# danieleschmidt/Graph-Hypernetwork-Forge

Measured on AMD Instinct MI355X. Metric: edges/s (HyperGNN forward), higher is better.
Workload: dtype f32; 1 GPU; synthetic uniform KG 1M nodes / 10M edges / 64 rel, hidden 128, L=3 (BASELINE config 3); nodes=1000000, edges=10000000, relations=64, hidden_dim=128, layers=3, text_dim=64, plan=cached (warm), launch=one C-ABI call per kernel, parallelism=single GPU

## Files before the change

graph-hypernetwork-forge_amd/csrc/message_bx.hip:

```cpp
#include "common.h"

#include <type_traits>

namespace ghf {

typedef float f32x4 __attribute__((ext_vector_type(4)));
typedef int i32x4 __attribute__((ext_vector_type(4)));
typedef int i32x2 __attribute__((ext_vector_type(2)));
typedef float f32x2 __attribute__((ext_vector_type(2)));
typedef _Float16 f16x8 __attribute__((ext_vector_type(8)));
typedef _Float16 f16x4 __attribute__((ext_vector_type(4)));
typedef __attribute__((address_space(3))) void* lptr_t;

template <class T>
__device__ __forceinline__ const T* bx_at(const void* base, uint32_t byte_off) {
    return (const T*)((const char*)base + byte_off);
}

__device__ __forceinline__ int lds_ld_b32(unsigned addr) {
    int v;
    asm volatile("ds_read_b32 %0, %1\n\ts_waitcnt lgkmcnt(0)" : "=&v"(v) : "v"(addr) : "memory");
    return v;
}
__device__ __forceinline__ void lds_ld_b32_x2(unsigned a0, unsigned a1, int& v0, int& v1) {
    asm volatile("ds_read_b32 %0, %2\n\tds_read_b32 %1, %3\n\ts_waitcnt lgkmcnt(0)" : "=&v"(v0), "=&v"(v1) : "v"(a0), "v"(a1) : "memory");
}
__device__ __forceinline__ void lds_ld_b32_x6(const unsigned (&a)[6], int (&v)[6]) {
    asm volatile("ds_read_b32 %0, %6\n\tds_read_b32 %1, %7\n\tds_read_b32 %2, %8\n\tds_read_b32 %3, %9\n\tds_read_b32 %4, %10\n\t"
                 "ds_read_b32 %5, %11\n\ts_waitcnt lgkmcnt(0)"
                 : "=&v"(v[0]), "=&v"(v[1]), "=&v"(v[2]), "=&v"(v[3]), "=&v"(v[4]), "=&v"(v[5])
                 : "v"(a[0]), "v"(a[1]), "v"(a[2]), "v"(a[3]), "v"(a[4]), "v"(a[5]) : "memory");
}
__device__ __forceinline__ void lds_ld_b32_x10(const unsigned (&a)[10], int (&v)[10]) {
    asm volatile("ds_read_b32 %0, %10\n\tds_read_b32 %1, %11\n\tds_read_b32 %2, %12\n\tds_read_b32 %3, %13\n\tds_read_b32 %4, %14\n\t"
                 "ds_read_b32 %5, %15\n\tds_read_b32 %6, %16\n\tds_read_b32 %7, %17\n\tds_read_b32 %8, %18\n\tds_read_b32 %9, %19\n\t"
                 "s_waitcnt lgkmcnt(0)"
                 : "=&v"(v[0]), "=&v"(v[1]), "=&v"(v[2]), "=&v"(v[3]), "=&v"(v[4]), "=&v"(v[5]), "=&v"(v[6]), "=&v"(v[7]), "=&v"(v[8]), "=&v"(v[9])
                 : "v"(a[0]), "v"(a[1]), "v"(a[2]), "v"(a[3]), "v"(a[4]), "v"(a[5]), "v"(a[6]), "v"(a[7]), "v"(a[8]), "v"(a[9]) : "memory");
}
__device__ __forceinline__ void lds_ld_b64_x2(unsigned a0, unsigned a1, f32x2& v0, f32x2& v1) {
    asm volatile("ds_read_b64 %0, %2\n\tds_read_b64 %1, %3\n\ts_waitcnt lgkmcnt(0)" : "=&v"(v0), "=&v"(v1) : "v"(a0), "v"(a1) : "memory");
}
__device__ __forceinline__ void lds_st_b32(unsigned addr, int v) { asm volatile("ds_write_b32 %0, %1" ::"v"(addr), "v"(v) : "memory"); }
__device__ __forceinline__ void lds_st_b64(unsigned addr, f32x2 v) { asm volatile("ds_write_b64 %0, %1" ::"v"(addr), "v"(v) : "memory"); }
__device__ __forceinline__ void lds_st_b128(unsigned addr, f32x4 v) { asm volatile("ds_write_b128 %0, %1" ::"v"(addr), "v"(v) : "memory"); }
#define BX_LGKM0() asm volatile("s_waitcnt lgkmcnt(0)" ::: "memory")
__device__ __forceinline__ int opaque_lane(int lane) {
    int z;
    asm volatile("v_mov_b32 %0, 0" : "=v"(z));
    return lane + z;
}

__device__ __forceinline__ int fresh_lane() {
    int z;
    asm volatile("v_mov_b32 %0, 0" : "=v"(z));
    return (int)__builtin_amdgcn_mbcnt_hi(~0u, __builtin_amdgcn_mbcnt_lo(~0u, (unsigned)z));
}

template <class T> __device__ __forceinline__ T bx_tail_ld(const T* p) { return __builtin_nontemporal_load(p); }
template <class T> __device__ __forceinline__ void bx_tail_st(T* p, T v) { __builtin_nontemporal_store(v, p); }
#define BX_IDX_WAIT "s_nop 3\n\t"
constexpr int BX_AD = 2, BX_TGB = 3;

template <int D> struct BxCfg;
template <> struct BxCfg<128> {
    static constexpr int NPW = 96, CR = 76;
    static constexpr int BN = 4 * NPW;
    static constexpr int MTC = (CR + 15) / 16;
    static constexpr bool DEFER = true;
    static constexpr size_t LDS = (size_t)4 * 2 * CR * 256 + 4 * (4 * 16 * MTC + 4) * 4 + 1024 + 512 + 64;
};
template <> struct BxCfg<64> {
    static constexpr int NPW = 48, CR = 64;
    static constexpr int BN = 4 * NPW;
    static constexpr int MTC = (CR + 15) / 16;
    static constexpr bool DEFER = false;
    static constexpr size_t LDS = (size_t)4 * 2 * CR * 128 + 4 * (4 * 16 * MTC + 4) * 4 + 1024 + 512 + 64;
};

typedef float f32x32 __attribute__((ext_vector_type(32)));
typedef float f32x16 __attribute__((ext_vector_type(16)));
#define BX_PIN_128(s) "+{v[64:95]}"(s[0]), "+{v[96:127]}"(s[1]), "+{v[128:159]}"(s[2]), "+{v[160:191]}"(s[3]), "+{v[192:223]}"(s[4]), "+{v[224:255]}"(s[5])
#define BX_PIN_64(s) "+{v[64:79]}"(s[0]), "+{v[80:95]}"(s[1]), "+{v[96:111]}"(s[2])

struct BxChunk { int r; int e0; int rows; };

template <int GB_, int NV_> struct BxTailSt {
    static constexpr int GB = GB_, NV = NV_;
    f32x4 x[GB_][NV_];
    int deg[GB_];
    float gm[4 * NV_], bt[4 * NV_];
};
constexpr int BX_TCG = 8;

template <int D, int SKIP>
__global__ __launch_bounds__(512, D == 64 ? 4 : 2) void message_bx_kernel(
    const float* __restrict__ h, const void* __restrict__ h_split, int64_t N, const uint32_t* __restrict__ sorted_key,
    const int32_t* __restrict__ sorted_src, const int32_t* __restrict__ chunk_tab,
    const int32_t* __restrict__ item_tab, int64_t item0, float* __restrict__ partial,
    const int32_t* __restrict__ indeg, int R,
    const void* __restrict__ Wsplit, const float* __restrict__ bias,
    const float* __restrict__ gamma, const float* __restrict__ beta, float eps,
    int64_t row0, int64_t row_end, float* __restrict__ h_out, void* __restrict__ h_split_out, int no_tail,
    int32_t* __restrict__ range_flag, float* __restrict__ agg_out) {
    using C = BxCfg<D>;
    constexpr bool SWAP1 = SKIP == 1;
    constexpr int skip = SWAP1 ? 2 : SKIP;
    constexpr int P0_IDS = SWAP1 ? 3 : 2;
    constexpr int P0_HALF = SWAP1 ? 1 : 0;
    constexpr int BN = C::BN, MTC = C::MTC, CR = C::CR, NPW = C::NPW;
    constexpr bool DEFER = C::DEFER;
    constexpr int NWV = 8, TW = 4;
    constexpr int KS = D / 32;
    constexpr int NKS = 2 * KS;
    constexpr int NT = D / 16;
    constexpr int NTW = NT / TW;
    constexpr int NPL = 2;
    constexpr int ROWB = D * 2;
    constexpr int PLANE = CR * ROWB;
    constexpr int TILE = NPL * PLANE;
    constexpr int HROW = NPL * D * 2;
    constexpr int CRP = 16 * MTC;
    constexpr int MSTR = 4 * CRP + 4;
    constexpr int PL = D / 64;
    constexpr int TUP = D == 128 ? 32 : 16;
    constexpr int NSV = NPW * PL / TUP;
    constexpr int RPP = 1024 / ROWB;
    constexpr int LPR = 64 / RPP;
    constexpr int RBN = CR / RPP;
    constexpr int CPL = D / 16;
    constexpr int RBW = (RBN + TW - 1) / TW;
    constexpr int RPH = (CR + TW - 1) / TW;
    static_assert((NTW == 2 || NTW == 1) && CR % RPP == 0 && RPH <= 64 && NPW * TW == BN && (NPW * PL) % TUP == 0 && NPW * PL <= 192 &&
                      NPW % 2 == 0 && (BN / 2) % 4 == 0 && CR <= 128 && NSV <= 6 && (D == 128 || D == 64), "bad config");
    auto akey = [](int row) -> int { return D == 128 ? (row & 15) : ((row >> 1) & 7); };
    constexpr unsigned META_OFF = 4 * TILE,
                       DUMMY_OFF = META_OFF + 4 * MSTR * 4, ZERO_OFF = DUMMY_OFF + 1024,
                       FLAG_OFF = ZERO_OFF + 512;
    auto tile_of = [](int j) -> unsigned { return (unsigned)(j & 3) * (unsigned)TILE; };

    extern __shared__ __attribute__((aligned(16))) char smem[];
    const unsigned lds0 = (unsigned)(size_t)(lptr_t)smem;

    const int tid = threadIdx.x, lane = tid & 63;
    const int w = __builtin_amdgcn_readfirstlane(tid >> 6);
    const bool helper = w >= TW;
    const int tw = w & 3;
    const int q = lane >> 4, c16 = lane & 15;
    const i32x4 item = *(const i32x4*)(item_tab + 4 * (size_t)(item0 + blockIdx.x));
    const int64_t blk = __builtin_amdgcn_readfirstlane(item[0]);
    const int slot = __builtin_amdgcn_readfirstlane(item[3]);
    const int64_t node0 = blk * BN;
    const int nrows = (int)((row_end - node0) < BN ? (row_end - node0) : BN);
    const uint32_t seg0 = (uint32_t)(blk * R);
    const int c_begin = __builtin_amdgcn_readfirstlane(item[1]);
    const int c_end = __builtin_amdgcn_readfirstlane(item[2]);
    const int nchunks = c_end - c_begin;
    int vzero;
    asm volatile("v_mov_b32 %0, 0" : "=v"(vzero));

    auto load_desc = [&](int k) -> i32x2 {
        const int c = c_begin + (k < nchunks ? k : 0) + vzero;
        return *bx_at<i32x2>(chunk_tab, (uint32_t)c * 8u);
    };
    auto decode = [&](i32x2 d) -> BxChunk {
        const int w0 = __builtin_amdgcn_readfirstlane(d[0]), w1 = __builtin_amdgcn_readfirstlane(d[1]);
        return BxChunk{w1 >> 8, w0, w1 & 127};
    };
    auto meta_off = [&](int j) -> unsigned { return META_OFF + (unsigned)(j & 3) * (MSTR * 4); };
    const uint32_t hsc_off = (uint32_t)((uint64_t)N * HROW);

    constexpr int HN = BN / 2, HPW = NPW / 2;
    auto tail_half = [&](int half, auto gb_c) __attribute__((always_inline)) {
        const float* acc_lds = (const float*)smem;
        constexpr int CS = 64;
        const int sub = lane >> 4, c0 = 4 * (lane & 15);
        constexpr int NV = CPL / 4;
        auto node_of = [&](int v) -> int { return (v / HPW) * NPW + half * HPW + (v % HPW); };
        auto row_sum = [&](float v) -> float {
            v += dpp_take<0xB1, 0xF>(v);
            v += dpp_take<0x4E, 0xF>(v);
            v += dpp_take<0x141, 0xF>(v);
            v += dpp_take<0x140, 0xF>(v);
            return v;
        };
        auto row_max = [&](float v) -> float {
            v = fmaxf(v, dpp_take<0xB1, 0xF>(v));
            v = fmaxf(v, dpp_take<0x4E, 0xF>(v));
            v = fmaxf(v, dpp_take<0x141, 0xF>(v));
            v = fmaxf(v, dpp_take<0x140, 0xF>(v));
            return v;
        };
        constexpr int NG = HN / 4;
        if (slot >= 0) {
            float* __restrict__ ps = partial + (size_t)slot * BN * D;
            for (int g = w; g < NG; g += NWV) {
                const int v = 4 * g + sub;
                float* __restrict__ o = ps + (size_t)node_of(v) * D + c0;
#pragma unroll
                for (int i = 0; i < NV; ++i) *(f32x4*)(o + CS * i) = *(const f32x4*)(acc_lds + v * D + c0 + CS * i);
            }
            return;
        }
        float gm[CPL], bt[CPL];
#pragma unroll
        for (int c = 0; c < CPL; ++c) {
            gm[c] = no_tail ? 1.f : gamma[c0 + CS * (c >> 2) + (c & 3)];
            bt[c] = no_tail ? 0.f : beta[c0 + CS * (c >> 2) + (c & 3)];
        }
        constexpr int GB = decltype(gb_c)::value;
        for (int g0 = w; g0 < NG; g0 += NWV * GB) {
            f32x4 x[GB][NV];
            float inv[GB];
            int deg[GB];
#pragma unroll
            for (int gb = 0; gb < GB; ++gb) {
                const int g = g0 + gb * NWV;
                const int nl = node_of(4 * (g < NG ? g : NG - 1) + sub);
                const int64_t node = node0 + (nl < nrows ? nl : nrows - 1);
                deg[gb] = indeg[node];
                const float* __restrict__ hp = h + (size_t)node * D + c0;
#pragma unroll
                for (int i = 0; i < NV; ++i)
                    x[gb][i] = (no_tail && !(no_tail & GHF_FLAG_ADD_H)) ? (f32x4){0.f, 0.f, 0.f, 0.f} : bx_tail_ld((const f32x4*)(hp + CS * i));
            }
            __builtin_amdgcn_sched_barrier(0);
#pragma unroll
            for (int gb = 0; gb < GB; ++gb) inv[gb] = (no_tail & GHF_FLAG_RAW_SUM) ? 1.0f : 1.0f / (float)(deg[gb] > 1 ? deg[gb] : 1);
#pragma unroll
            for (int gb = 0; gb < GB; ++gb) {
                const int g = g0 + gb * NWV;
                const int v = 4 * (g < NG ? g : NG - 1) + sub;
                const int nl = node_of(v);
                const bool live = g < NG && nl < nrows;
                f32x4 a[NV];
#pragma unroll
                for (int i = 0; i < NV; ++i) a[i] = *(const f32x4*)(acc_lds + v * D + c0 + CS * i);
                if (agg_out && live) {
                    float* __restrict__ o = agg_out + (size_t)(node0 + nl) * D + c0;
#pragma unroll
                    for (int i = 0; i < NV; ++i) bx_tail_st((f32x4*)(o + CS * i), a[i] * inv[gb]);
                }
                float y[CPL];
                float s = 0.f;
#pragma unroll
                for (int c = 0; c < CPL; ++c) {
                    const float av = a[c >> 2][c & 3] * inv[gb];
                    y[c] = no_tail ? av + x[gb][c >> 2][c & 3] : fmaxf(av + x[gb][c >> 2][c & 3], 0.f);
                    s += y[c];
                }
                if (!no_tail) {
                    const float mean = row_sum(s) * (1.0f / D);
                    float var = 0.f;
#pragma unroll
                    for (int c = 0; c < CPL; ++c) { const float t = y[c] - mean; var += t * t; }
                    const float rstd = 1.0f / sqrtf(row_sum(var) * (1.0f / D) + eps);
#pragma unroll
                    for (int c = 0; c < CPL; ++c) y[c] = (y[c] - mean) * rstd * gm[c] + bt[c];
                }
                float up = 1.f;
                if (h_split_out) {
                    float mx = 0.f;
#pragma unroll
                    for (int c = 0; c < CPL; ++c) mx = fmaxf(mx, fabsf(y[c]));
                    const int sh = split2h_shift(row_max(mx));
                    up = pow2f(sh);
                    if ((lane & 15) == 0 && live) *(float*)((char*)h_split_out + (size_t)hsc_off + (size_t)(node0 + nl) * 4) = pow2f(-sh);
                }
                if (live) {
                    float* __restrict__ o = h_out + (size_t)(node0 + nl) * D + c0;
#pragma unroll
                    for (int i = 0; i < NV; ++i) bx_tail_st((f32x4*)(o + CS * i), (f32x4){y[4 * i], y[4 * i + 1], y[4 * i + 2], y[4 * i + 3]});
                    if (h_split_out) {
                        _Float16* __restrict__ sp = (_Float16*)h_split_out + (size_t)(node0 + nl) * (NPL * D) + c0;
                        _Float16 hi[CPL], lo[CPL];
#pragma unroll
                        for (int c = 0; c < CPL; ++c) split2h(y[c] * up, hi[c], lo[c]);
                        if constexpr (CPL == 8 && CS == 4) {
                            *(f16x8*)sp = (f16x8){hi[0], hi[1], hi[2], hi[3], hi[4], hi[5], hi[6], hi[7]};
                            *(f16x8*)(sp + D) = (f16x8){lo[0], lo[1], lo[2], lo[3], lo[4], lo[5], lo[6], lo[7]};
                        } else if constexpr (CPL == 8) {
#pragma unroll
                            for (int i = 0; i < 2; ++i) {
                                bx_tail_st((f16x4*)(sp + CS * i), (f16x4){hi[4 * i], hi[4 * i + 1], hi[4 * i + 2], hi[4 * i + 3]});
                                bx_tail_st((f16x4*)(sp + D + CS * i), (f16x4){lo[4 * i], lo[4 * i + 1], lo[4 * i + 2], lo[4 * i + 3]});
                            }
                        } else {
                            bx_tail_st((f16x4*)sp, (f16x4){hi[0], hi[1], hi[2], hi[3]});
                            bx_tail_st((f16x4*)(sp + D), (f16x4){lo[0], lo[1], lo[2], lo[3]});
                        }
                    }
                }
                if (h_split_out) {
                    int tiny = 0, nz = 0;
#pragma unroll
                    for (int c = 0; c < CPL; ++c) { tiny += range_tiny(y[c] * up); nz += y[c] != 0.f; }
                    if (__ballot(tiny != 0)) {
                        tiny = (int)row_sum((float)tiny);
                        nz = (int)row_sum((float)nz);
                        if ((lane & 15) == 0 && live) range_raise(range_flag, GHF_RANGE_ROWS, tiny, nz);
                    }
                }
            }
        }
    };

    auto tail_issue = [&](int half, auto& st, int gfirst, auto gend_c) __attribute__((always_inline)) {
        using St = typename std::remove_reference<decltype(st)>::type;
        constexpr int GB = St::GB, NV = St::NV, CS = 64;
        static_assert(NV * 4 == CPL && 4 * GB <= decltype(gend_c)::value, "one batch holds all of the wave's groups");
        if (slot >= 0) return;
        const int tl = fresh_lane(), sub = tl >> 4, c0 = 4 * (tl & 15);
        const bool no_x = no_tail && !(no_tail & GHF_FLAG_ADD_H);
        const __amdgpu_buffer_rsrc_t rsG = __builtin_amdgcn_make_buffer_rsrc((void*)gamma, 0, no_tail ? 0 : D * 4, 0x00020000);
        const __amdgpu_buffer_rsrc_t rsB = __builtin_amdgcn_make_buffer_rsrc((void*)beta, 0, no_tail ? 0 : D * 4, 0x00020000);
        const __amdgpu_buffer_rsrc_t rsX = __builtin_amdgcn_make_buffer_rsrc(
            (void*)h, 0, no_x ? 0 : (int)(uint32_t)((uint64_t)N * D * 4), 0x00020000);
#pragma unroll
        for (int c = 0; c < CPL; ++c) {
            st.gm[c] = __builtin_bit_cast(float, __builtin_amdgcn_raw_buffer_load_b32(rsG, (c0 + CS * (c >> 2) + (c & 3)) * 4, 0, 0));
            st.bt[c] = __builtin_bit_cast(float, __builtin_amdgcn_raw_buffer_load_b32(rsB, (c0 + CS * (c >> 2) + (c & 3)) * 4, 0, 0));
        }
#pragma unroll
        for (int gb = 0; gb < GB; ++gb) {
            const int v = 4 * (gfirst + 4 * gb) + sub;
            const int nl = (v / HPW) * NPW + half * HPW + (v % HPW);
            const int64_t node = node0 + (nl < nrows ? nl : nrows - 1);
            st.deg[gb] = indeg[node];
#pragma unroll
            for (int i = 0; i < NV; ++i)
                st.x[gb][i] = __builtin_bit_cast(f32x4, __builtin_amdgcn_raw_buffer_load_b128(
                    rsX, (int)(((uint32_t)node * D + c0 + CS * i) * 4u), 0, 2 ));
        }
        __builtin_amdgcn_sched_barrier(0);
    };
    auto tail_rows = [&](int half, auto& st, int gfirst, auto gend_c) __attribute__((always_inline)) {
        using St = typename std::remove_reference<decltype(st)>::type;
        constexpr int GB = St::GB, NV = St::NV, gend = decltype(gend_c)::value, CS = 64;
        __builtin_amdgcn_s_waitcnt(0x0F70);
        const float* acc_lds = (const float*)smem;
        const int tl = fresh_lane(), sub = tl >> 4, c0 = 4 * (tl & 15);
        auto node_of = [&](int v) -> int { return (v / HPW) * NPW + half * HPW + (v % HPW); };
        auto row_sum = [&](float v) -> float {
            v += dpp_take<0xB1, 0xF>(v);
            v += dpp_take<0x4E, 0xF>(v);
            v += dpp_take<0x141, 0xF>(v);
            v += dpp_take<0x140, 0xF>(v);
            return v;
        };
        auto row_max = [&](float v) -> float {
            v = fmaxf(v, dpp_take<0xB1, 0xF>(v));
            v = fmaxf(v, dpp_take<0x4E, 0xF>(v));
            v = fmaxf(v, dpp_take<0x141, 0xF>(v));
            v = fmaxf(v, dpp_take<0x140, 0xF>(v));
            return v;
        };
        if (slot >= 0) {
            float* __restrict__ ps = partial + (size_t)slot * BN * D;
            for (int g = gfirst; g < gend; g += 4) {
                const int v = 4 * g + sub;
                float* __restrict__ o = ps + (size_t)node_of(v) * D + c0;
#pragma unroll
                for (int i = 0; i < NV; ++i) *(f32x4*)(o + CS * i) = *(const f32x4*)(acc_lds + v * D + c0 + CS * i);
            }
            return;
        }
        float inv[GB];
#pragma unroll
        for (int gb = 0; gb < GB; ++gb) inv[gb] = (no_tail & GHF_FLAG_RAW_SUM) ? 1.0f : 1.0f / (float)(st.deg[gb] > 1 ? st.deg[gb] : 1);
#pragma unroll
        for (int gb = 0; gb < GB; ++gb) {
            const int v = 4 * (gfirst + 4 * gb) + sub;
            const int nl = node_of(v);
            const bool live = nl < nrows;
            f32x4 a[NV];
#pragma unroll
            for (int i = 0; i < NV; ++i) a[i] = *(const f32x4*)(acc_lds + v * D + c0 + CS * i);
            if (agg_out && live) {
                float* __restrict__ o = agg_out + (size_t)(node0 + nl) * D + c0;
#pragma unroll
                for (int i = 0; i < NV; ++i) bx_tail_st((f32x4*)(o + CS * i), a[i] * inv[gb]);
            }
            float y[CPL];
            float s = 0.f;
#pragma unroll
            for (int c = 0; c < CPL; ++c) {
                const float av = a[c >> 2][c & 3] * inv[gb];
                y[c] = no_tail ? av + st.x[gb][c >> 2][c & 3] : fmaxf(av + st.x[gb][c >> 2][c & 3], 0.f);
                s += y[c];
            }
            if (!no_tail) {
                const float mean = row_sum(s) * (1.0f / D);
                float var = 0.f;
#pragma unroll
                for (int c = 0; c < CPL; ++c) { const float t = y[c] - mean; var += t * t; }
                const float rstd = 1.0f / sqrtf(row_sum(var) * (1.0f / D) + eps);
#pragma unroll
                for (int c = 0; c < CPL; ++c) y[c] = (y[c] - mean) * rstd * st.gm[c] + st.bt[c];
            }
            float up = 1.f;
            if (h_split_out) {
                float mx = 0.f;
#pragma unroll
                for (int c = 0; c < CPL; ++c) mx = fmaxf(mx, fabsf(y[c]));
                const int sh = split2h_shift(row_max(mx));
                up = pow2f(sh);
                if ((tl & 15) == 0 && live) *(float*)((char*)h_split_out + (size_t)hsc_off + (size_t)(node0 + nl) * 4) = pow2f(-sh);
            }
            if (live) {
                float* __restrict__ o = h_out + (size_t)(node0 + nl) * D + c0;
#pragma unroll
                for (int i = 0; i < NV; ++i) bx_tail_st((f32x4*)(o + CS * i), (f32x4){y[4 * i], y[4 * i + 1], y[4 * i + 2], y[4 * i + 3]});
                if (h_split_out) {
                    _Float16* __restrict__ sp = (_Float16*)h_split_out + (size_t)(node0 + nl) * (NPL * D) + c0;
                    _Float16 hi[CPL], lo[CPL];
#pragma unroll
                    for (int c = 0; c < CPL; ++c) split2h(y[c] * up, hi[c], lo[c]);
#pragma unroll
                    for (int i = 0; i < NV; ++i) {
                        bx_tail_st((f16x4*)(sp + CS * i), (f16x4){hi[4 * i], hi[4 * i + 1], hi[4 * i + 2], hi[4 * i + 3]});
                        bx_tail_st((f16x4*)(sp + D + CS * i), (f16x4){lo[4 * i], lo[4 * i + 1], lo[4 * i + 2], lo[4 * i + 3]});
                    }
                }
            }
            if (h_split_out) {
                int tiny = 0, nz = 0;
#pragma unroll
                for (int c = 0; c < CPL; ++c) { tiny += range_tiny(y[c] * up); nz += y[c] != 0.f; }
                if (__ballot(tiny != 0)) {
                    tiny = (int)row_sum((float)tiny);
                    nz = (int)row_sum((float)nz);
                    if ((tl & 15) == 0 && live) range_raise(range_flag, GHF_RANGE_ROWS, tiny, nz);
                }
            }
        }
    };
    auto tail_barrier = [&]() __attribute__((always_inline)) {
        BX_LGKM0();
        __builtin_amdgcn_s_barrier();
        asm volatile("" ::: "memory");
    };
    constexpr int TNG = BN / 2 / 4;
    constexpr int TCG = BX_TCG, THG = TNG / 4 - TCG;
    static_assert(D != 128 || (TNG % 4 == 0 && TCG >= 1 && THG >= 1 && 9 * THG + 2 * CPL <= 96),
                  "the helpers' operands of a half fit the registers its dump freed");
    std::integral_constant<int, TNG> c_tng;
    std::integral_constant<int, 4 * TCG> c_cend;

    if (helper) {
        typename std::conditional<D == 128, f32x32, f32x16>::type sm[NSV];
#pragma unroll
        for (int k = 0; k < NSV; ++k)
#pragma unroll
            for (int i = 0; i < TUP; ++i) sm[k][i] = 0.f;
        if constexpr (D == 128) asm volatile("" : BX_PIN_128(sm)); else asm volatile("" : BX_PIN_64(sm));
        const int hw = tw;
        const __amdgpu_buffer_rsrc_t rsH = __builtin_amdgcn_make_buffer_rsrc((void*)h_split, 0, (int)hsc_off, 0x00020000);
        struct Words { int src; int key; };
        struct Scales { float u; float v; };
        auto load_words = [&](const BxChunk& c, int ln) -> Words {
            const int mrow = hw * RPH + (ln < RPH ? ln : RPH - 1);
            const int rc = mrow < c.rows ? mrow : c.rows - 1;
            const uint32_t eo = (uint32_t)(c.e0 + rc) * 4u;
            return Words{*bx_at<int>(sorted_src, eo), *bx_at<int>(sorted_key, eo)};
        };
        auto dst_of = [&](const BxChunk& c, const Words& wd) -> uint32_t {
            const uint32_t kbase = (seg0 + (uint32_t)c.r) * (uint32_t)BN;
            return (uint32_t)node0 + ((uint32_t)wd.key - kbase);
        };
        auto load_scales = [&](const BxChunk& c, const Words& wd) -> Scales {
            const uint32_t nu = (uint32_t)(wd.src & SRC_MASK), nv = dst_of(c, wd);
            return Scales{*bx_at<float>(h_split, hsc_off + nu * 4u), *bx_at<float>(h_split, hsc_off + nv * 4u)};
        };
        auto publish = [&](int j, const BxChunk& c, const Words& wd, const Scales& sc, int ln) {
            const unsigned m = lds0 + meta_off(j);
            const int mrow = hw * RPH + (ln < RPH ? ln : RPH - 1);
            if (ln < RPH && mrow < CRP) {
                lds_st_b32(m + 4 * mrow, __float_as_int(sc.u));
                lds_st_b32(m + 4 * (CRP + mrow), __float_as_int(sc.v));
                lds_st_b32(m + 4 * (2 * CRP + mrow), wd.src & SRC_MASK);
                lds_st_b32(m + 4 * (3 * CRP + mrow), (int)dst_of(c, wd));
            }
            if (hw == 0 && ln == 0) lds_st_b32(m + 4 * (4 * CRP), c.rows);
        };
        static_assert(RBW <= 6, "ids of a tile: one batched read");
        auto id_addr = [&](int j, int which , int i, int lane) -> unsigned {
            return lds0 + meta_off(j) + 4 * (which * CRP) + 4 * (RPP * (hw + TW * (i < RBW ? i : 0)) + lane / LPR);
        };
        auto dma_ids = [&](int j, int which, int lane, int (&id)[6]) {
            unsigned ia[6];
#pragma unroll
            for (int i = 0; i < 6; ++i) ia[i] = id_addr(j, which, i, lane);
            lds_ld_b32_x6(ia, id);
        };
        auto dma_issue = [&](unsigned tile_off, int rows, int lane, const int (&id)[6]) {
#pragma unroll
            for (int i_ = 0; i_ < RBW; ++i_) {
                const int i = i_;
                const int rb = hw + TW * i, row = RPP * rb + lane / LPR;
                if (RPP * rb >= rows) continue;
                const int g = (lane & (LPR - 1)) ^ akey(row);
                const int voff = row < rows ? (int)((uint32_t)id[i] * (uint32_t)HROW) + (g << 4) : (int)0xFFFFF000u;
                const unsigned dst = rb < RBN ? tile_off + (unsigned)rb * 1024u : DUMMY_OFF;
#pragma unroll
                for (int pl = 0; pl < NPL; ++pl) {
                    const unsigned d = __builtin_amdgcn_readfirstlane(dst + (rb < RBN ? pl * PLANE : 0));
                    __builtin_amdgcn_raw_ptr_buffer_load_lds(rsH, (lptr_t)(smem + d), 16, voff + pl * ROWB, 0, 0, 0);
                }
            }
        };
        auto dma_tile = [&](unsigned tile_off, int j, int which, const BxChunk& c, int lane) {
            int id[6];
            dma_ids(j, which, lane, id);
            dma_issue(tile_off, c.rows, lane, id);
        };
        struct FoldPlan { int n0, n1, ra, cnt; };
        auto fold_plan = [&](int j, int rows, int lane) __attribute__((always_inline)) -> FoldPlan {
            const unsigned dd = lds0 + meta_off(j) + 4 * (3 * CRP);
            int d0, d1;
            lds_ld_b32_x2(dd + 4 * lane, dd + 4 * (lane + 64 < CRP ? lane + 64 : CRP - 1), d0, d1);
            const int base = (int)node0 + hw * NPW;
            const int n0 = d0 - base, n1 = d1 - base;
            const unsigned long long q0 = __ballot(lane < rows && (unsigned)n0 < (unsigned)NPW);
            const unsigned long long q1 = __ballot(lane + 64 < rows && (unsigned)n1 < (unsigned)NPW);
            const int cnt = __builtin_popcountll(q0) + __builtin_popcountll(q1);
            const int ra = q0 ? (int)__builtin_ctzll(q0) : 64 + (q1 ? (int)__builtin_ctzll(q1) : 0);
            return FoldPlan{n0, n1, ra, cnt};
        };
        auto fold_rows = [&](int j, const FoldPlan& fp, int lane) __attribute__((always_inline)) {
            const unsigned Y = lds0 + tile_of(j - 1);
            const int ra = fp.ra, cnt = fp.cnt;
            const unsigned zrow = lds0 + ZERO_OFF + (unsigned)(PL * 4 * lane), lb = (unsigned)(PL * 4 * lane);
            typedef typename std::conditional<D == 128, f32x2, float>::type yv_t;
            constexpr int FB = 4;
            auto issue = [&](yv_t (&y)[FB], int r0) __attribute__((always_inline)) {
                unsigned a[FB];
#pragma unroll
                for (int i = 0; i < FB; ++i) {
                    const int rr = ra + r0 + i;
                    a[i] = r0 + i < cnt ? Y + (unsigned)rr * (D * 4) + (lb ^ (unsigned)(((rr >> 2) & 1) << 7)) : zrow;
                }
                if constexpr (D == 128)
                    asm volatile("ds_read_b64 %0, %4\n\tds_read_b64 %1, %5\n\tds_read_b64 %2, %6\n\tds_read_b64 %3, %7"
                                 : "=&v"(y[0]), "=&v"(y[1]), "=&v"(y[2]), "=&v"(y[3]) : "v"(a[0]), "v"(a[1]), "v"(a[2]), "v"(a[3]) : "memory");
                else
                    asm volatile("ds_read_b32 %0, %4\n\tds_read_b32 %1, %5\n\tds_read_b32 %2, %6\n\tds_read_b32 %3, %7"
                                 : "=&v"(y[0]), "=&v"(y[1]), "=&v"(y[2]), "=&v"(y[3]) : "v"(a[0]), "v"(a[1]), "v"(a[2]), "v"(a[3]) : "memory");
            };
            auto add_rows = [&](yv_t (&y)[FB], int r0, bool behind) __attribute__((always_inline)) {
                if (behind) asm volatile("s_waitcnt lgkmcnt(4)" : "+v"(y[0]), "+v"(y[1]), "+v"(y[2]), "+v"(y[3])::"memory");
                else asm volatile("s_waitcnt lgkmcnt(0)" : "+v"(y[0]), "+v"(y[1]), "+v"(y[2]), "+v"(y[3])::"memory");
                int ix[FB];
#pragma unroll
                for (int i = 0; i < FB; ++i) {
                    const int rr = ra + r0 + i;
                    const int a = __builtin_amdgcn_readlane(fp.n0, rr & 63), b = __builtin_amdgcn_readlane(fp.n1, rr & 63);
                    ix[i] = r0 + i < cnt ? PL * (rr < 64 ? a : b) : 0;
                }
                int keep;
#define BX_ROW128(i) "s_set_gpr_idx_idx %[i" #i "]\n\tv_pk_add_f32 v[64:65], %[y" #i "], v[64:65]\n\t"
#define BX_ROW64(i) "s_set_gpr_idx_idx %[i" #i "]\n\tv_add_f32 v64, %[y" #i "], v64\n\t"
#define BX_ROW_OPS [i0] "s"(ix[0]), [i1] "s"(ix[1]), [i2] "s"(ix[2]), [i3] "s"(ix[3]), [y0] "v"(y[0]), [y1] "v"(y[1]), [y2] "v"(y[2]), [y3] "v"(y[3])
                if constexpr (D == 128)
                    asm volatile("s_mov_b32 %[kp], m0\n\ts_set_gpr_idx_on %[i0], 0xa\n\t" BX_IDX_WAIT "v_pk_add_f32 v[64:65], %[y0], v[64:65]\n\t"
                                 BX_ROW128(1) BX_ROW128(2) BX_ROW128(3)
                                 "s_set_gpr_idx_off\n\t" BX_IDX_WAIT "s_mov_b32 m0, %[kp]"
                                 : BX_PIN_128(sm), [kp] "=&s"(keep) : BX_ROW_OPS);
                else
                    asm volatile("s_mov_b32 %[kp], m0\n\ts_set_gpr_idx_on %[i0], 0xa\n\t" BX_IDX_WAIT "v_add_f32 v64, %[y0], v64\n\t"
                                 BX_ROW64(1) BX_ROW64(2) BX_ROW64(3)
                                 "s_set_gpr_idx_off\n\t" BX_IDX_WAIT "s_mov_b32 m0, %[kp]"
                                 : BX_PIN_64(sm), [kp] "=&s"(keep) : BX_ROW_OPS);
#undef BX_ROW128
#undef BX_ROW64
#undef BX_ROW_OPS
            };
            for (int g = 0; g < cnt; g += 2 * FB) {
                yv_t ya[FB], yb[FB];
                issue(ya, g);
                issue(yb, g + FB);
                add_rows(ya, g, true);
                add_rows(yb, g + FB, false);
            }
        };
        auto wait_flags = [&](unsigned flags, int v) {
            for (;;) {
                i32x4 f;
                asm volatile("ds_read_b128 %0, %1\n\ts_waitcnt lgkmcnt(0)" : "=&v"(f) : "v"(flags) : "memory");
                const int lo = min(min(f[0], f[1]), min(f[2], f[3]));
                if (__builtin_amdgcn_readfirstlane(lo) >= v) break;
                __builtin_amdgcn_s_sleep(1);
            }
        };
        auto wait_flags2 = [&](unsigned fa, unsigned fb, int v) {
            for (;;) {
                i32x4 f, g;
                asm volatile("ds_read_b128 %0, %2\n\tds_read_b128 %1, %3\n\ts_waitcnt lgkmcnt(0)" : "=&v"(f), "=&v"(g) : "v"(fa), "v"(fb) : "memory");
                const int lo = min(min(min(f[0], f[1]), min(f[2], f[3])), min(min(g[0], g[1]), min(g[2], g[3])));
                if (__builtin_amdgcn_readfirstlane(lo) >= v) break;
                __builtin_amdgcn_s_sleep(1);
            }
        };

        BxChunk ch[5];
        Words wdP{0, 0}, wdN{0, 0}, wdL{0, 0};
        Scales scP{1.f, 1.f}, scN{1.f, 1.f};
        i32x2 d5{0, 0};
        if (hw == 0)
#pragma unroll
            for (int i = 0; i < 3; ++i)
                if (lane + 64 * i < 128 + 16) lds_st_b32(lds0 + ZERO_OFF + 4 * (lane + 64 * i), 0);
        int prev_rows = 1;
        if (nchunks > 0) {
            i32x2 dd[5];
#pragma unroll
            for (int j = 0; j < 5; ++j) dd[j] = load_desc(j);
#pragma unroll
            for (int j = 0; j < 5; ++j) ch[j] = decode(dd[j]);
            Words wd[4];
            Scales sc[3];
#pragma unroll
            for (int j = 0; j < 4; ++j) wd[j] = load_words(ch[j], lane);
#pragma unroll
            for (int j = 0; j < 3; ++j) sc[j] = load_scales(ch[j], wd[j]);
#pragma unroll
            for (int j = 0; j < 2; ++j) publish(j, ch[j], wd[j], sc[j], lane);
            wdP = wd[2];
            scP = sc[2];
            wdN = wd[3];
        }
        BX_LGKM0();
        __builtin_amdgcn_s_barrier();
        if (nchunks > 0) {
            if (!(skip & 1)) dma_tile(tile_of(0), 0, P0_IDS, ch[0], lane);
            if (!(skip & 2)) dma_tile(tile_of(-1), 0, 3, ch[0], lane);
            asm volatile("s_waitcnt vmcnt(0)" ::: "memory");
        }
        int sid[6] = {0, 0, 0, 0, 0, 0};
        if (nchunks > 0 && !(skip & 1)) dma_ids(1, P0_IDS, lane, sid);
        for (int k = 0; k < nchunks; ++k) {
            __builtin_amdgcn_s_barrier();
            const int l0 = opaque_lane(lane);
            if (k > 0) {
                wdP = wdN;
                scP = scN;
                wdN = wdL;
#pragma unroll
                for (int j = 0; j < 4; ++j) ch[j] = ch[j + 1];
                ch[4] = decode(d5);
                asm volatile("" : "+v"(wdP.src), "+v"(wdP.key), "+v"(scP.u), "+v"(scP.v), "+v"(wdN.src), "+v"(wdN.key));
            }
            publish(k + 2, ch[2], wdP, scP, l0);
            if (!(skip & 1)) dma_issue(tile_of(k + 1), ch[1].rows, l0, sid);
            BX_LGKM0();
            if (lane == 0) lds_st_b32(lds0 + FLAG_OFF + 4 * hw, k + 1);
            if (k > 0) {
                const FoldPlan fp = fold_plan(k - 1, prev_rows, l0);
                if (DEFER) wait_flags(lds0 + FLAG_OFF + 16, k);
                fold_rows(k - 1, fp, l0);
            }
            int did[6];
            if (!(skip & 2)) {
                dma_ids(k + 1, 3, opaque_lane(lane), did);
                wait_flags2(lds0 + FLAG_OFF, lds0 + FLAG_OFF + 32, k + 1);
            } else {
                wait_flags(lds0 + FLAG_OFF, k + 1);
            }
            const int l1 = opaque_lane(lane);
            scN = load_scales(ch[3], wdN);
            wdL = load_words(ch[4], l1);
            d5 = load_desc(k + 5);
            if (!(skip & 2)) dma_issue(tile_of(k), ch[1].rows, l1, did);
            prev_rows = ch[0].rows;
            if (!(skip & 1)) dma_ids(k + 2, P0_IDS, l1, sid);
            asm volatile("s_waitcnt vmcnt(0)" ::: "memory");
            BX_LGKM0();
        }
        __builtin_amdgcn_s_barrier();
        if (nchunks > 0) {
            const int le = opaque_lane(lane);
            fold_rows(nchunks - 1, fold_plan(nchunks - 1, prev_rows, le), le);
        }
        asm volatile("s_waitcnt vmcnt(0)" ::: "memory");
        BX_LGKM0();
        if constexpr (D == 128) asm volatile("" : BX_PIN_128(sm)); else asm volatile("" : BX_PIN_64(sm));
        auto dump_half = [&](auto half_c) __attribute__((always_inline)) {
            constexpr int H = decltype(half_c)::value;
            float* __restrict__ o = (float*)smem + (size_t)(hw * HPW) * D + (D == 128 ? 32 * (lane >> 4) + (lane & 15) : lane);
#pragma unroll
            for (int i = 0; i < HPW; ++i)
#pragma unroll
                for (int e = 0; e < PL; ++e) {
                    const int reg = PL * (H * HPW + i) + e;
                    o[i * D + 16 * e] = sm[reg / TUP][reg % TUP];
                }
        };
        __syncthreads();
        dump_half(std::integral_constant<int, 0>{});
        if constexpr (D == 128) {
            const int gf = 4 * TCG + hw;
            BxTailSt<THG, CPL / 4> st;
            tail_issue(0, st, gf, c_tng);
            tail_barrier();
            tail_rows(0, st, gf, c_tng);
            tail_issue(1, st, gf, c_tng);
            tail_barrier();
            dump_half(std::integral_constant<int, 1>{});
            tail_barrier();
            tail_rows(1, st, gf, c_tng);
        } else {
            BX_LGKM0();
            __syncthreads();
            tail_half(0, std::integral_constant<int, 1>{});
            __syncthreads();
            dump_half(std::integral_constant<int, 1>{});
            BX_LGKM0();
            __syncthreads();
            tail_half(1, std::integral_constant<int, BX_TGB>{});
        }
    } else {
        const uint32_t wsc_off = (uint32_t)((uint64_t)R * 2 * D * D * (NPL * 2));
        const __amdgpu_buffer_rsrc_t rsW = __builtin_amdgcn_make_buffer_rsrc((void*)Wsplit, 0, (int)wsc_off, 0x00020000);
        auto b_soff = [&](int r, int ph, int t) -> int {
            return __builtin_amdgcn_readfirstlane((((r * NT + tw * NTW + t) * NKS + ph * KS) * NPL) * 1024);
        };
        const int lane16 = lane * 16;
        i32x4 b[KS][NTW][NPL];
        auto load_b_step = [&](int r, int ph, int j) {
#pragma unroll
            for (int t = 0; t < NTW; ++t)
#pragma unroll
                for (int pl = 0; pl < NPL; ++pl)
                    b[j][t][pl] = __builtin_amdgcn_raw_buffer_load_b128(rsW, lane16 + pl * 1024, b_soff(r, ph, t) + j * (NPL * 1024), 0);
        };
        f32x4 acc[MTC][NTW];
        const int arow = c16 * ROWB;
        constexpr int AD = BX_AD;
        static_assert(AD <= MTC - 2, "the prefetched positions are row tiles 0 .. AD-1 of the first k-step in every instance");
        i32x4 apre[AD][NPL];
        auto lda_from = [&](const char* Abuf, int j, int m, i32x4 (&dst)[NPL]) __attribute__((always_inline)) {
            const char* src = Abuf + arow + (((4 * j + q) ^ akey(c16)) << 4) + m * 16 * ROWB;
#pragma unroll
            for (int pl = 0; pl < NPL; ++pl) dst[pl] = *(const i32x4*)(src + pl * PLANE);
        };
        auto prefetch_a = [&](const char* Abuf) __attribute__((always_inline)) {
#pragma unroll
            for (int p = 0; p < AD; ++p) lda_from(Abuf, 0, p, apre[p]);
        };
        auto compute_stage = [&](auto mt_c, auto pre_c, int ph, bool first, const char* Abuf, const int* meta, float wscale, int r_next, int ph_next,
                                 const float (&bias_v)[NTW], auto&& after_k) __attribute__((always_inline)) {
            constexpr int MT = decltype(mt_c)::value;
            constexpr bool PRE = decltype(pre_c)::value;
            f32x4 part[MTC][NTW];
#pragma unroll
            for (int m = 0; m < MT; ++m)
#pragma unroll
                for (int t = 0; t < NTW; ++t) part[m][t] = (f32x4){0.f, 0.f, 0.f, 0.f};
            f32x4 sc[MTC];
            i32x4 a[AD + 1][NPL];
            auto lda = [&](int j, int m, i32x4 (&dst)[NPL]) { lda_from(Abuf, j, m, dst); };
#pragma unroll
            for (int p = 0; p < AD && p < KS * MT; ++p) {
                if constexpr (PRE) {
#pragma unroll
                    for (int pl = 0; pl < NPL; ++pl) a[p][pl] = apre[p][pl];
                } else {
                    lda(p / MT, p % MT, a[p]);
                }
            }
#pragma unroll
            for (int j = 0; j < KS; ++j) {
                if (j == KS - 1) {
#pragma unroll
                    for (int m = 0; m < MT; ++m) sc[m] = *(const f32x4*)(meta + ph * CRP + m * 16 + 4 * q);
                }
#pragma unroll
                for (int m = 0; m < MT; ++m) {
                    const int p = j * MT + m, cur = p % (AD + 1);
                    if (p + AD < KS * MT) lda((p + AD) / MT, (p + AD) % MT, a[(p + AD) % (AD + 1)]);
#pragma unroll
                    for (int t = 0; t < NTW; ++t) {
                        auto fma = [&](int pa, int pb) {
                            part[m][t] = __builtin_amdgcn_mfma_f32_16x16x32_f16(__builtin_bit_cast(f16x8, a[cur][pa]),
                                                                                __builtin_bit_cast(f16x8, b[j][t][pb]),
                                                                                part[m][t], 0, 0, 0);
                        };
                        fma(1, 0); fma(0, 1);
                        fma(0, 0);
                    }
                }
                __builtin_amdgcn_sched_barrier(0);
                load_b_step(r_next, ph_next, j);
                __builtin_amdgcn_sched_barrier(0);
            }
            after_k();
#pragma unroll
            for (int m = 0; m < MT; ++m) {
#pragma unroll
                for (int s = 0; s < 4; ++s) {
                    const float f = sc[m][s] * wscale;
#pragma unroll
                    for (int t = 0; t < NTW; ++t) acc[m][t][s] = fmaf(part[m][t][s], f, first ? bias_v[t] : acc[m][t][s]);
                }
            }
#pragma unroll
            for (int m = MT; m < MTC; ++m)
#pragma unroll
                for (int t = 0; t < NTW; ++t) acc[m][t] = (f32x4){0.f, 0.f, 0.f, 0.f};
        };
        auto stage_for = [&](int mt, auto pre_c, int ph, bool first, const char* Abuf, const int* meta, float wscale, int r_next, int ph_next,
                             const float (&bias_v)[NTW], auto&& after_k) __attribute__((always_inline)) {
            static_assert(MTC >= 3, "three compute_stage instances");
            if (mt >= MTC) compute_stage(std::integral_constant<int, MTC>{}, pre_c, ph, first, Abuf, meta, wscale, r_next, ph_next, bias_v, after_k);
            else if (mt == MTC - 1) compute_stage(std::integral_constant<int, MTC - 1>{}, pre_c, ph, first, Abuf, meta, wscale, r_next, ph_next, bias_v, after_k);
            else compute_stage(std::integral_constant<int, MTC - 2>{}, pre_c, ph, first, Abuf, meta, wscale, r_next, ph_next, bias_v, after_k);
        };
        const unsigned yoff = (unsigned)(4 * q) * (D * 4) + (unsigned)((((NTW == 2 ? 32 * tw + 2 * c16 : 16 * tw + c16)) ^ ((q & 1) << 5)) * 4);
        auto write_rows = [&](int mt, unsigned ytile) __attribute__((always_inline)) {
            const unsigned ybase = lds0 + ytile + yoff;
#pragma unroll
            for (int m = 0; m < MTC; ++m) {
                if (m >= mt) continue;
                if (16 * m + 16 > CR && 16 * m + 4 * q >= CR) continue;
#pragma unroll
                for (int s = 0; s < 4; ++s) {
                    if constexpr (NTW == 2)
                        asm volatile("ds_write_b64 %0, %1 offset:%2" ::"v"(ybase), "v"((f32x2){acc[m][0][s], acc[m][NTW - 1][s]}),
                                     "n"((16 * m + s) * (D * 4)) : "memory");
                    else
                        asm volatile("ds_write_b32 %0, %1 offset:%2" ::"v"(ybase), "v"(acc[m][0][s]), "n"((16 * m + s) * (D * 4)) : "memory");
                }
            }
        };

        const int ph_first = (skip & 1) ? 1 : P0_HALF;
        BxChunk ch{0, 0, 1};
        i32x2 dn{0, 0};
        float bias_v[NTW] = {}, bias_n[NTW] = {}, wscale = 1.f, wscale_n = 1.f;
        auto load_rel_words = [&](int r, float& ws, float (&bv)[NTW]) {
            ws = *bx_at<float>(Wsplit, wsc_off + (uint32_t)(r + vzero) * 4u);
#pragma unroll
            for (int t = 0; t < NTW; ++t) bv[t] = *bx_at<float>(bias, (uint32_t)(r * D + (tw * NTW + t) * 16 + c16) * 4u);
        };
        int mt_prev = 0;
        if (nchunks > 0) {
            ch = decode(load_desc(0));
            dn = load_desc(1);
            load_rel_words(ch.r, wscale, bias_v);
#pragma unroll
            for (int j = 0; j < KS; ++j) load_b_step(ch.r, ph_first, j);
        }
        __syncthreads();
        for (int k = 0; k < nchunks; ++k) {
            const int mt = (ch.rows + 15) >> 4;
            const int* meta = (const int*)(smem + meta_off(k));
            __syncthreads();
            if (DEFER && k > 0) {
                write_rows(mt_prev, tile_of(k - 2));
                BX_LGKM0();
                if (lane == 0) lds_st_b32(lds0 + FLAG_OFF + 16 + 4 * tw, k);
            }
            const BxChunk nx = decode(dn);
            constexpr bool PRE1 = false;
            static_assert(!PRE1, "the hook has no flag words of its own any more: wait_landed spins on words that mean something else (a hung CU)");
            auto wait_landed = [&]() __attribute__((always_inline)) {
                for (;;) {
                    i32x4 f;
                    asm volatile("ds_read_b128 %0, %1\n\ts_waitcnt lgkmcnt(0)" : "=&v"(f) : "v"(lds0 + FLAG_OFF) : "memory");
                    const int lo = min(min(f[0], f[1]), min(f[2], f[3]));
                    if (__builtin_amdgcn_readfirstlane(lo) >= k + 1) break;
                    __builtin_amdgcn_s_sleep(1);
                }
            };
            auto next_pre = [&]() __attribute__((always_inline)) {
                if (PRE1) {
                    wait_landed();
                    prefetch_a(smem + tile_of(k - 1));
                }
            };
            auto no_after = []() {};
            if (!(skip & 1))
                stage_for(mt, std::false_type{}, P0_HALF, true, smem + tile_of(k), meta, wscale, (skip & 2) ? nx.r : ch.r, (skip & 2) ? P0_HALF : 1, bias_v, next_pre);
            if (!(skip & 2) && lane == 0) lds_st_b32(lds0 + FLAG_OFF + 32 + 4 * tw, k + 1);
            dn = load_desc(k + 2);
            load_rel_words(nx.r, wscale_n, bias_n);
            if (skip & 1) {
#pragma unroll
                for (int m = 0; m < MTC; ++m)
#pragma unroll
                    for (int t = 0; t < NTW; ++t) acc[m][t] = (f32x4){bias_v[t], bias_v[t], bias_v[t], bias_v[t]};
            }
            if (!(skip & 2)) stage_for(mt, std::false_type{}, 1, false, smem + tile_of(k - 1), meta, wscale, nx.r, ph_first, bias_v, no_after);
            const bool stage_now = !DEFER || k + 1 == nchunks;
            if (stage_now) {
                const unsigned fw = DEFER ? FLAG_OFF + 48 : FLAG_OFF + 16;
                const int fv = DEFER ? 1 : k + 1;
                if (lane == 0) lds_st_b32(lds0 + fw + 4 * tw, fv);
                for (;;) {
                    i32x4 f;
                    asm volatile("ds_read_b128 %0, %1\n\ts_waitcnt lgkmcnt(0)" : "=&v"(f) : "v"(lds0 + fw) : "memory");
                    const int lo = min(min(f[0], f[1]), min(f[2], f[3]));
                    if (__builtin_amdgcn_readfirstlane(lo) >= fv) break;
                    __builtin_amdgcn_s_sleep(1);
                }
                write_rows(mt, tile_of(k - 1));
            }
            mt_prev = mt;
            ch = nx;
            wscale = wscale_n;
#pragma unroll
            for (int t = 0; t < NTW; ++t) bias_v[t] = bias_n[t];
            BX_LGKM0();
        }
        __syncthreads();
        if constexpr (D == 128) {
            BxTailSt<TCG, CPL / 4> st;
            tail_issue(0, st, tw, c_cend);
            tail_barrier();
            tail_barrier();
            tail_rows(0, st, tw, c_cend);
            tail_issue(1, st, tw, c_cend);
            tail_barrier();
            tail_barrier();
            tail_rows(1, st, tw, c_cend);
        } else {
            for (int half = 0; half < 2; ++half) {
                __syncthreads();
                __syncthreads();
                tail_half(half, std::integral_constant<int, BX_TGB>{});
            }
        }
    }
}

template <int D>
static int launch_bx_for(const MsgArgs& a, hipStream_t stream) {
    using C = BxCfg<D>;
    constexpr size_t lds = C::LDS;
    static_assert(lds <= 160 * 1024, "LDS budget");
    static_assert((size_t)(C::BN / 2) * D * 4 <= (size_t)3 * 2 * C::CR * (D * 2), "the tail's dump of half a block must fit three whole tiles of the ring");
    GHF_REQUIRE(a.block_nodes == C::BN, "message(bx): plan block_nodes=%d, kernel for d=%d needs %d", a.block_nodes, D, C::BN);
    GHF_REQUIRE(a.wlayout == GHF_WLAYOUT_SPLIT2H, "message(bx): weights must be in SPLIT2H layout");
    GHF_REQUIRE(a.chunk_tab && a.item_tab && a.blk_item_off, "message(bx): the plan's chunk / item tables are missing");
    GHF_REQUIRE(a.h_split, "message(bx): h_split is missing (ghf_split_rows)");
    const int64_t row_end = a.row0 + a.rows;
    GHF_REQUIRE(row_end == a.N || row_end % C::BN == 0, "message(bx): row range must end on a block boundary or at N");
    if (a.rows <= 0) return GHF_OK;
    GHF_REQUIRE((uint64_t)a.N * (D * 4 + 4) <= 0xFFFFF000ull && (uint64_t)a.E * 4 < (1ull << 32) &&
                    (uint64_t)a.R * (2 * D * D * 4 + 4) < (1ull << 32),
                "message(bx): 32-bit byte offsets need N*(4d+4) <= 4 GiB - 4 KiB, E*4 and R*(8d*d+4) below 4 GiB");
    GHF_REQUIRE(a.n_items >= cdiv(a.rows, C::BN), "message(bx): n_items=%lld is fewer than the blocks of the row range", (long long)a.n_items);
    GHF_REQUIRE(a.n_items == cdiv(a.rows, C::BN) || a.partial, "message(bx): split blocks need the `partial` scratch");
    const int skip = ((a.flags & GHF_FLAG_ZERO_SRC) ? 1 : 0) | ((a.flags & GHF_FLAG_ZERO_DST) ? 2 : 0);
    const size_t lds_dyn = lds;
    auto go = [&](auto skip_c) {
        constexpr int S = decltype(skip_c)::value;
        GHF_SET_MAX_LDS((message_bx_kernel<D, S>), lds_dyn);
        message_bx_kernel<D, S><<<(unsigned)a.n_items, 512, lds_dyn, stream>>>(a.h, a.h_split, a.N, a.sorted_key, a.sorted_src, a.chunk_tab, a.item_tab,
                                                                          a.item0, a.partial, a.indeg, a.R, a.W_msg, a.bias, a.ln_gamma,
                                                                          a.ln_beta, a.ln_eps, a.row0, row_end, a.h_out, a.h_split_out,
                                                                          a.flags & (GHF_FLAG_NO_TAIL | GHF_FLAG_RAW_SUM | GHF_FLAG_ADD_H), range_flag_ptr(), a.agg_out);
        return GHF_OK;
    };
    if (skip == 1) go(std::integral_constant<int, 1>{});
    else if (skip == 2) go(std::integral_constant<int, 2>{});
    else go(std::integral_constant<int, 0>{});
    GHF_LAUNCH_CHECK();
    if (a.n_items > cdiv(a.rows, C::BN)) return launch_combine_split(a, stream);
    return GHF_OK;
}

__global__ __launch_bounds__(256) void split2h_rows_kernel(const float* __restrict__ h, int64_t N, int64_t row0, int64_t rows,
                                                           int d, char* __restrict__ out, int32_t* __restrict__ range_flag) {
    const int lane = threadIdx.x & 63;
    const int64_t i = (int64_t)blockIdx.x * 4 + (threadIdx.x >> 6);
    if (i >= rows) return;
    const int64_t row = row0 + i;
    const float* __restrict__ src = h + row * d;
    float mx = 0.f;
    for (int k = lane; k < d; k += 64) mx = fmaxf(mx, fabsf(src[k]));
    const int sh = split2h_shift(wave_absmax(mx));
    const float up = pow2f(sh);
    _Float16* __restrict__ dst = (_Float16*)(out + row * (4 * (int64_t)d));
    int tiny = 0, nz = 0;
    for (int k = lane; k < d; k += 64) {
        _Float16 hi, lo;
        const float xs = src[k] * up;
        split2h(xs, hi, lo);
        dst[k] = hi;
        dst[d + k] = lo;
        tiny += __popcll(__ballot(range_tiny(xs)));
        nz += __popcll(__ballot(xs != 0.f));
    }
    if (lane == 0) {
        *(float*)(out + N * (4 * (int64_t)d) + row * 4) = pow2f(-sh);
        range_raise(range_flag, GHF_RANGE_ROWS, tiny, nz);
    }
}

int launch_split2h_rows(const float* h, int64_t N, int d, int64_t row0, int64_t rows, void* h_split, hipStream_t stream) {
    if (rows <= 0) return GHF_OK;
    GHF_REQUIRE(cdiv(rows, 4) < (1ll << 31), "split_rows: too many rows per launch");
    split2h_rows_kernel<<<(unsigned)cdiv(rows, 4), 256, 0, stream>>>(h, N, row0, rows, d, (char*)h_split, range_flag_ptr());
    GHF_LAUNCH_CHECK();
    return GHF_OK;
}

bool message_bx_config(int d, int* block_nodes, int* chunk_rows, int* split_chunks) {
    if (d != 128 && d != 64) return false;
    *block_nodes = d == 128 ? BxCfg<128>::BN : BxCfg<64>::BN;
    *chunk_rows = d == 128 ? BxCfg<128>::CR : BxCfg<64>::CR;
    *split_chunks = 128;
    return true;
}

bool message_bx_owns(int d, int block_nodes) {
    return (d == 128 && block_nodes == BxCfg<128>::BN) || (d == 64 && block_nodes == BxCfg<64>::BN);
}

int launch_message_bx(const MsgArgs& a, hipStream_t stream) {
    if (a.d == 128) return launch_bx_for<128>(a, stream);
    if (a.d == 64) return launch_bx_for<64>(a, stream);
    return set_err(GHF_EUNSUPPORTED, "message(bx): no kernel for d=%d", a.d);
}

}
```

Measured before the change: 1.078 billion edges/s.

## Split fold across DMA issue phases and merge flag poll into fold plan read

The per-chunk fold of the previous tile is split into two parts: the first rows are folded before the next DMA descriptors are issued, and the rest after. The flag check for staged data is merged into the same LDS read batch as the fold-plan indices, so the explicit wait runs only when the data is not ready yet. The producer-side landed-flag store moves into the stage hook so consumers are released earlier. The aim is to hide DMA issue latency and flag-polling stalls behind fold work, at the cost of a more fragile cross-wave handshake and an extra s_nop per indexed add.

```diff
diff --git a/graph-hypernetwork-forge_amd/csrc/message_bx.hip b/graph-hypernetwork-forge_amd/csrc/message_bx.hip
--- a/graph-hypernetwork-forge_amd/csrc/message_bx.hip
+++ b/graph-hypernetwork-forge_amd/csrc/message_bx.hip
@@ -61,6 +61,7 @@
 template <class T> __device__ __forceinline__ void bx_tail_st(T* p, T v) { __builtin_nontemporal_store(v, p); }
 #define BX_IDX_WAIT "s_nop 3\n\t"
 constexpr int BX_AD = 2, BX_TGB = 3;
+constexpr int BX_FSPLIT = 8;
 
 template <int D> struct BxCfg;
 template <> struct BxCfg<128> {
@@ -515,10 +516,19 @@
             dma_issue(tile_off, c.rows, lane, id);
         };
         struct FoldPlan { int n0, n1, ra, cnt; };
-        auto fold_plan = [&](int j, int rows, int lane) __attribute__((always_inline)) -> FoldPlan {
+        auto fold_plan = [&](int j, int rows, int lane, int staged, bool* ready) __attribute__((always_inline)) -> FoldPlan {
             const unsigned dd = lds0 + meta_off(j) + 4 * (3 * CRP);
+            const unsigned a0 = dd + 4 * lane, a1 = dd + 4 * (lane + 64 < CRP ? lane + 64 : CRP - 1);
             int d0, d1;
-            lds_ld_b32_x2(dd + 4 * lane, dd + 4 * (lane + 64 < CRP ? lane + 64 : CRP - 1), d0, d1);
+            if (staged > 0) {
+                i32x4 f;
+                asm volatile("ds_read_b32 %0, %3\n\tds_read_b32 %1, %4\n\tds_read_b128 %2, %5\n\ts_waitcnt lgkmcnt(0)"
+                             : "=&v"(d0), "=&v"(d1), "=&v"(f) : "v"(a0), "v"(a1), "v"(lds0 + FLAG_OFF + 16) : "memory");
+                *ready = __builtin_amdgcn_readfirstlane(min(min(f[0], f[1]), min(f[2], f[3]))) >= staged;
+            } else {
+                lds_ld_b32_x2(a0, a1, d0, d1);
+                *ready = true;
+            }
             const int base = (int)node0 + hw * NPW;
             const int n0 = d0 - base, n1 = d1 - base;
             const unsigned long long q0 = __ballot(lane < rows && (unsigned)n0 < (unsigned)NPW);
@@ -527,7 +537,7 @@
             const int ra = q0 ? (int)__builtin_ctzll(q0) : 64 + (q1 ? (int)__builtin_ctzll(q1) : 0);
             return FoldPlan{n0, n1, ra, cnt};
         };
-        auto fold_rows = [&](int j, const FoldPlan& fp, int lane) __attribute__((always_inline)) {
+        auto fold_rows = [&](int j, const FoldPlan& fp, int lane, int g_begin, int g_end) __attribute__((always_inline)) {
             const unsigned Y = lds0 + tile_of(j - 1);
             const int ra = fp.ra, cnt = fp.cnt;
             const unsigned zrow = lds0 + ZERO_OFF + (unsigned)(PL * 4 * lane), lb = (unsigned)(PL * 4 * lane);
@@ -564,18 +574,18 @@
                 if constexpr (D == 128)
                     asm volatile("s_mov_b32 %[kp], m0\n\ts_set_gpr_idx_on %[i0], 0xa\n\t" BX_IDX_WAIT "v_pk_add_f32 v[64:65], %[y0], v[64:65]\n\t"
                                  BX_ROW128(1) BX_ROW128(2) BX_ROW128(3)
-                                 "s_set_gpr_idx_off\n\t" BX_IDX_WAIT "s_mov_b32 m0, %[kp]"
+                                 "s_set_gpr_idx_off\n\t" BX_IDX_WAIT "s_mov_b32 m0, %[kp]\n\ts_nop 0"
                                  : BX_PIN_128(sm), [kp] "=&s"(keep) : BX_ROW_OPS);
                 else
                     asm volatile("s_mov_b32 %[kp], m0\n\ts_set_gpr_idx_on %[i0], 0xa\n\t" BX_IDX_WAIT "v_add_f32 v64, %[y0], v64\n\t"
                                  BX_ROW64(1) BX_ROW64(2) BX_ROW64(3)
-                                 "s_set_gpr_idx_off\n\t" BX_IDX_WAIT "s_mov_b32 m0, %[kp]"
+                                 "s_set_gpr_idx_off\n\t" BX_IDX_WAIT "s_mov_b32 m0, %[kp]\n\ts_nop 0"
                                  : BX_PIN_64(sm), [kp] "=&s"(keep) : BX_ROW_OPS);
 #undef BX_ROW128
 #undef BX_ROW64
 #undef BX_ROW_OPS
             };
-            for (int g = 0; g < cnt; g += 2 * FB) {
+            for (int g = g_begin; g < cnt && g < g_end; g += 2 * FB) {
                 yv_t ya[FB], yb[FB];
                 issue(ya, g);
                 issue(yb, g + FB);
@@ -654,10 +664,12 @@
             if (!(skip & 1)) dma_issue(tile_of(k + 1), ch[1].rows, l0, sid);
             BX_LGKM0();
             if (lane == 0) lds_st_b32(lds0 + FLAG_OFF + 4 * hw, k + 1);
+            FoldPlan fp{0, 0, 0, 0};
             if (k > 0) {
-                const FoldPlan fp = fold_plan(k - 1, prev_rows, l0);
-                if (DEFER) wait_flags(lds0 + FLAG_OFF + 16, k);
-                fold_rows(k - 1, fp, l0);
+                bool staged;
+                fp = fold_plan(k - 1, prev_rows, l0, DEFER ? k : 0, &staged);
+                if (DEFER && !staged) wait_flags(lds0 + FLAG_OFF + 16, k);
+                fold_rows(k - 1, fp, l0, 0, BX_FSPLIT);
             }
             int did[6];
             if (!(skip & 2)) {
@@ -671,6 +683,7 @@
             wdL = load_words(ch[4], l1);
             d5 = load_desc(k + 5);
             if (!(skip & 2)) dma_issue(tile_of(k), ch[1].rows, l1, did);
+            fold_rows(k - 1, fp, l1, BX_FSPLIT, CR + 8);
             prev_rows = ch[0].rows;
             if (!(skip & 1)) dma_ids(k + 2, P0_IDS, l1, sid);
             asm volatile("s_waitcnt vmcnt(0)" ::: "memory");
@@ -679,7 +692,8 @@
         __builtin_amdgcn_s_barrier();
         if (nchunks > 0) {
             const int le = opaque_lane(lane);
-            fold_rows(nchunks - 1, fold_plan(nchunks - 1, prev_rows, le), le);
+            bool staged;
+            fold_rows(nchunks - 1, fold_plan(nchunks - 1, prev_rows, le, 0, &staged), le, 0, CR + 8);
         }
         asm volatile("s_waitcnt vmcnt(0)" ::: "memory");
         BX_LGKM0();
@@ -877,11 +891,11 @@
                     wait_landed();
                     prefetch_a(smem + tile_of(k - 1));
                 }
+                if (!(skip & 2) && lane == 0) lds_st_b32(lds0 + FLAG_OFF + 32 + 4 * tw, k + 1);
             };
             auto no_after = []() {};
             if (!(skip & 1))
                 stage_for(mt, std::false_type{}, P0_HALF, true, smem + tile_of(k), meta, wscale, (skip & 2) ? nx.r : ch.r, (skip & 2) ? P0_HALF : 1, bias_v, next_pre);
-            if (!(skip & 2) && lane == 0) lds_st_b32(lds0 + FLAG_OFF + 32 + 4 * tw, k + 1);
             dn = load_desc(k + 2);
             load_rel_words(nx.r, wscale_n, bias_n);
             if (skip & 1) {
```

Result: faster. 1.103 billion edges/s, median of 6 (+2.3%).
